# YulioTech/Yulio-Raytracer

Hardware: AMD Instinct MI355X
Metric: Mrays/s (Sponza stand-in 2048^2 64spp, closest+shadow queries) (higher is better)
Workload: dtype f32

## Files before the change

### yulio-raytracer_amd/csrc/device/bvh_build.cpp

```cpp
#include "bvh_build.h"

#include <float.h>
#include <math.h>
#include <stdlib.h>
#include <string.h>

#include <algorithm>
#include <stdexcept>

namespace yrt {

namespace {

struct Box {
  float lo[3], hi[3];
  void reset() {
    for (int k = 0; k < 3; ++k) { lo[k] = INFINITY; hi[k] = -INFINITY; }
  }
  void grow(const Box& b) {
    for (int k = 0; k < 3; ++k) { lo[k] = std::min(lo[k], b.lo[k]); hi[k] = std::max(hi[k], b.hi[k]); }
  }
  void growP(const float* p) {
    for (int k = 0; k < 3; ++k) { lo[k] = std::min(lo[k], p[k]); hi[k] = std::max(hi[k], p[k]); }
  }
  float area() const {
    const float dx = hi[0] - lo[0], dy = hi[1] - lo[1], dz = hi[2] - lo[2];
    if (!(dx >= 0 && dy >= 0 && dz >= 0)) return 0.f;
    return 2.f * (dx * dy + dy * dz + dz * dx);
  }
};

struct Prim {
  Box b;
  float c[3];
  int id;
};

struct Node2 {
  Box b[2];
  int idx[2], cnt[2];
};

struct Builder {
  std::vector<Prim> prims;
  std::vector<Node2> nodes;
#ifndef YRT_MAX_LEAF
#define YRT_MAX_LEAF 8
#endif
  int maxLeaf = YRT_MAX_LEAF;
#ifndef YRT_SAH_TRAV
#define YRT_SAH_TRAV 1.0f
#endif
  int medianDepth = 24;
  int maxDepthSeen = 0;

  Box bounds(int b, int e) const {
    Box bb;
    bb.reset();
    for (int i = b; i < e; ++i) bb.grow(prims[i].b);
    return bb;
  }

  int split(int b, int e, int depth, bool& makeLeaf) {
    const int n = e - b;
    makeLeaf = false;
    Box cb;
    cb.reset();
    for (int i = b; i < e; ++i) cb.growP(prims[i].c);
    int axis = 0;
    float ext = cb.hi[0] - cb.lo[0];
    for (int k = 1; k < 3; ++k)
      if (cb.hi[k] - cb.lo[k] > ext) { ext = cb.hi[k] - cb.lo[k]; axis = k; }
    if (!(ext > 0.f)) {
      if (n <= maxLeaf) { makeLeaf = true; return e; }
      return b + n / 2;
    }
    if (depth >= medianDepth) {
      const int m = b + n / 2;
      std::nth_element(prims.begin() + b, prims.begin() + m, prims.begin() + e,
                       [axis](const Prim& x, const Prim& y) { return x.c[axis] < y.c[axis]; });
      return m;
    }
    const int NB = 32;
    float bestCost = INFINITY;
    int bestAxis = -1, bestBin = -1;
    for (int ax = 0; ax < 3; ++ax) {
      const float lo = cb.lo[ax], hi = cb.hi[ax];
      if (!(hi > lo)) continue;
      const float scale = NB / (hi - lo);
      Box bb[NB];
      int cnt[NB] = {0};
      for (int k = 0; k < NB; ++k) bb[k].reset();
      for (int i = b; i < e; ++i) {
        int bin = std::min(NB - 1, (int)((prims[i].c[ax] - lo) * scale));
        cnt[bin]++;
        bb[bin].grow(prims[i].b);
      }
      float rightArea[NB];
      int rightCnt[NB];
      Box acc;
      acc.reset();
      int ac = 0;
      for (int k = NB - 1; k > 0; --k) {
        acc.grow(bb[k]);
        ac += cnt[k];
        rightArea[k] = acc.area();
        rightCnt[k] = ac;
      }
      acc.reset();
      ac = 0;
      for (int k = 0; k < NB - 1; ++k) {
        acc.grow(bb[k]);
        ac += cnt[k];
        if (ac == 0 || rightCnt[k + 1] == 0) continue;
        const float cost = acc.area() * ac + rightArea[k + 1] * rightCnt[k + 1];
        if (cost < bestCost) { bestCost = cost; bestAxis = ax; bestBin = k; }
      }
    }
    const float parentArea = bounds(b, e).area();
    const float leafCost = (float)n;
    const float splitCost = YRT_SAH_TRAV + (parentArea > 0.f ? bestCost / parentArea : (float)n);
    if (n <= maxLeaf && leafCost <= splitCost) { makeLeaf = true; return e; }
    if (bestAxis < 0) return b + n / 2;
    const float lo = cb.lo[bestAxis], hi = cb.hi[bestAxis];
    const float scale = NB / (hi - lo);
    auto mid = std::partition(prims.begin() + b, prims.begin() + e, [&](const Prim& p) {
      return std::min(NB - 1, (int)((p.c[bestAxis] - lo) * scale)) <= bestBin;
    });
    int m = (int)(mid - prims.begin());
    if (m <= b || m >= e) m = b + n / 2;
    return m;
  }

  void child(int b, int e, int depth, int& idx, int& cnt, Box& bb) {
    bb = bounds(b, e);
    const int n = e - b;
    if (n <= 2 && n < 32) { idx = b; cnt = n; return; }
    bool leaf = false;
    const int m = split(b, e, depth, leaf);
    if (leaf && n <= 31) { idx = b; cnt = n; return; }
    idx = inner(b, m, e, depth);
    cnt = 0;
  }

  int inner(int b, int m, int e, int depth) {
    if (depth > maxDepthSeen) maxDepthSeen = depth;
    const int ni = (int)nodes.size();
    nodes.emplace_back();
    int i0, c0, i1, c1;
    Box b0, b1;
    child(b, m, depth + 1, i0, c0, b0);
    child(m, e, depth + 1, i1, c1, b1);
    Node2& n = nodes[ni];
    n.b[0] = b0;
    n.b[1] = b1;
    n.idx[0] = i0; n.idx[1] = i1;
    n.cnt[0] = c0; n.cnt[1] = c1;
    return ni;
  }
};

#ifndef YRT_SBVH_ALPHA
#define YRT_SBVH_ALPHA 1e-5f
#endif
#ifndef YRT_SBVH_BUDGET
#define YRT_SBVH_BUDGET 0.5f
#endif
struct SRef {
  Box b;
  int id;
  float c(int k) const { return 0.5f * (b.lo[k] + b.hi[k]); }
};

Box clip_tri(const float* t, int axis, float lo, float hi) {
  Box r;
  r.reset();
  for (int e = 0; e < 3; ++e) {
    const float* p = t + 3 * e;
    const float* q = t + 3 * ((e + 1) % 3);
    const float pa = p[axis], qa = q[axis];
    if (pa >= lo && pa <= hi) r.growP(p);
    const float planes[2] = {lo, hi};
    for (float pl : planes) {
      if ((pa < pl && qa > pl) || (pa > pl && qa < pl)) {
        const double tt = ((double)pl - pa) / ((double)qa - pa);
        float x[3];
        for (int k = 0; k < 3; ++k) x[k] = (float)(p[k] + tt * ((double)q[k] - p[k]));
        x[axis] = pl;
        r.growP(x);
      }
    }
  }
  for (int k = 0; k < 3; ++k) {
    if (k == axis || !(r.hi[k] >= r.lo[k])) continue;
    const float pad = 4.0f * FLT_EPSILON * std::max(fabsf(r.lo[k]), fabsf(r.hi[k]));
    r.lo[k] -= pad;
    r.hi[k] += pad;
  }
  return r;
}

Box intersect(const Box& a, const Box& b) {
  Box r;
  for (int k = 0; k < 3; ++k) {
    r.lo[k] = std::max(a.lo[k], b.lo[k]);
    r.hi[k] = std::min(a.hi[k], b.hi[k]);
  }
  return r;
}

struct SplitBuilder {
  const std::vector<float>& v;
  std::vector<Node2> nodes;
  std::vector<int> leafIds;
  int maxLeaf = YRT_MAX_LEAF;
  int medianDepth = 24;
  float minOverlap = 0.f;
  size_t refBudget = 0, numRefs = 0;
  explicit SplitBuilder(const std::vector<float>& verts) : v(verts) {}

  static Box bounds(const std::vector<SRef>& r) {
    Box bb;
    bb.reset();
    for (const SRef& x : r) bb.grow(x.b);
    return bb;
  }

  void leaf(std::vector<SRef>& refs, int& idx, int& cnt) {
    idx = (int)leafIds.size();
    cnt = (int)refs.size();
    for (const SRef& x : refs) leafIds.push_back(x.id);
  }

  void child(std::vector<SRef>& refs, int depth, int& idx, int& cnt, Box& bb) {
    bb = bounds(refs);
    const int n = (int)refs.size();
    if (n <= 2) { leaf(refs, idx, cnt); return; }
    std::vector<SRef> L, R;
    const bool mkLeaf = split(refs, bb, depth, L, R);
    if (mkLeaf && n <= 31) { leaf(refs, idx, cnt); return; }
    if (mkLeaf) median(refs, bb, L, R);
    std::vector<SRef>().swap(refs);
    idx = inner(L, R, depth);
    cnt = 0;
  }

  int inner(std::vector<SRef>& L, std::vector<SRef>& R, int depth) {
    const int ni = (int)nodes.size();
    nodes.emplace_back();
    int i0, c0, i1, c1;
    Box b0, b1;
    child(L, depth + 1, i0, c0, b0);
    child(R, depth + 1, i1, c1, b1);
    Node2& nd = nodes[ni];
    nd.b[0] = b0;
    nd.b[1] = b1;
    nd.idx[0] = i0; nd.idx[1] = i1;
    nd.cnt[0] = c0; nd.cnt[1] = c1;
    return ni;
  }

  void median(std::vector<SRef>& refs, const Box& bb, std::vector<SRef>& L, std::vector<SRef>& R) {
    int axis = 0;
    for (int k = 1; k < 3; ++k)
      if (bb.hi[k] - bb.lo[k] > bb.hi[axis] - bb.lo[axis]) axis = k;
    const size_t m = refs.size() / 2;
    std::nth_element(refs.begin(), refs.begin() + m, refs.end(),
                     [axis](const SRef& x, const SRef& y) { return x.c(axis) < y.c(axis); });
    L.assign(refs.begin(), refs.begin() + m);
    R.assign(refs.begin() + m, refs.end());
  }

  bool split(std::vector<SRef>& refs, const Box& nodeBox, int depth, std::vector<SRef>& L, std::vector<SRef>& R) {
    const int n = (int)refs.size();
    Box cb;
    cb.reset();
    for (const SRef& x : refs) {
      const float c[3] = {x.c(0), x.c(1), x.c(2)};
      cb.growP(c);
    }
    if (depth >= medianDepth) {
      median(refs, cb, L, R);
      return false;
    }
    const int NB = 32;
    float objCost = INFINITY;
    int objAxis = -1, objBin = -1;
    Box objL, objR;
    for (int ax = 0; ax < 3; ++ax) {
      const float lo = cb.lo[ax], hi = cb.hi[ax];
      if (!(hi > lo)) continue;
      const float scale = NB / (hi - lo);
      Box bb[NB];
      int cnt[NB] = {0};
      for (int k = 0; k < NB; ++k) bb[k].reset();
      for (const SRef& x : refs) {
        const int bin = std::min(NB - 1, (int)((x.c(ax) - lo) * scale));
        cnt[bin]++;
        bb[bin].grow(x.b);
      }
      Box rightBox[NB];
      int rightCnt[NB];
      Box acc;
      acc.reset();
      int ac = 0;
      for (int k = NB - 1; k > 0; --k) {
        acc.grow(bb[k]);
        ac += cnt[k];
        rightBox[k] = acc;
        rightCnt[k] = ac;
      }
      acc.reset();
      ac = 0;
      for (int k = 0; k < NB - 1; ++k) {
        acc.grow(bb[k]);
        ac += cnt[k];
        if (ac == 0 || rightCnt[k + 1] == 0) continue;
        const float cost = acc.area() * ac + rightBox[k + 1].area() * rightCnt[k + 1];
        if (cost < objCost) {
          objCost = cost; objAxis = ax; objBin = k; objL = acc; objR = rightBox[k + 1];
        }
      }
    }
    float spCost = INFINITY;
    int spAxis = -1, spBin = -1;
    const float overlap = objAxis >= 0 ? intersect(objL, objR).area() : INFINITY;
    if (numRefs < refBudget && overlap > minOverlap) {
      for (int ax = 0; ax < 3; ++ax) {
        const float lo = nodeBox.lo[ax], hi = nodeBox.hi[ax];
        if (!(hi > lo)) continue;
        const float w = (hi - lo) / NB;
        Box bb[NB];
        int enter[NB] = {0}, exit[NB] = {0};
        for (int k = 0; k < NB; ++k) bb[k].reset();
        for (const SRef& x : refs) {
          const int b0 = std::max(0, std::min(NB - 1, (int)((x.b.lo[ax] - lo) / w)));
          const int b1 = std::max(b0, std::min(NB - 1, (int)((x.b.hi[ax] - lo) / w)));
          enter[b0]++;
          exit[b1]++;
          if (b0 == b1) {
            bb[b0].grow(x.b);
            continue;
          }
          const float* t = &v[(size_t)x.id * 9];
          for (int k = b0; k <= b1; ++k) {
            const float s0 = k == b0 ? x.b.lo[ax] : lo + k * w;
            const float s1 = k == b1 ? x.b.hi[ax] : lo + (k + 1) * w;
            const Box cbx = intersect(clip_tri(t, ax, s0, s1), x.b);
            if (cbx.hi[0] >= cbx.lo[0] && cbx.hi[1] >= cbx.lo[1] && cbx.hi[2] >= cbx.lo[2]) bb[k].grow(cbx);
          }
        }
        Box rightBox[NB];
        int rightCnt[NB];
        Box acc;
        acc.reset();
        int ac = 0;
        for (int k = NB - 1; k > 0; --k) {
          acc.grow(bb[k]);
          ac += exit[k];
          rightBox[k] = acc;
          rightCnt[k] = ac;
        }
        acc.reset();
        ac = 0;
        for (int k = 0; k < NB - 1; ++k) {
          acc.grow(bb[k]);
          ac += enter[k];
          if (ac == 0 || rightCnt[k + 1] == 0) continue;
          const float cost = acc.area() * ac + rightBox[k + 1].area() * rightCnt[k + 1];
          if (cost < spCost) { spCost = cost; spAxis = ax; spBin = k; }
        }
      }
    }
    const float parentArea = nodeBox.area();
    const float best = std::min(objCost, spCost);
    const float splitCost = YRT_SAH_TRAV + (parentArea > 0.f ? best / parentArea : (float)n);
    if (n <= maxLeaf && (float)n <= splitCost) return true;
    if (objAxis < 0 && spAxis < 0) return true;
    if (spAxis >= 0 && spCost < objCost) {
      const float lo = nodeBox.lo[spAxis], w = (nodeBox.hi[spAxis] - lo) / NB;
      const float plane = lo + (spBin + 1) * w;
      for (const SRef& x : refs) {
        if (x.b.hi[spAxis] <= plane) { L.push_back(x); continue; }
        if (x.b.lo[spAxis] >= plane) { R.push_back(x); continue; }
        const float* t = &v[(size_t)x.id * 9];
        const Box bl = intersect(clip_tri(t, spAxis, x.b.lo[spAxis], plane), x.b);
        const Box br = intersect(clip_tri(t, spAxis, plane, x.b.hi[spAxis]), x.b);
        const bool okL = bl.hi[0] >= bl.lo[0] && bl.hi[1] >= bl.lo[1] && bl.hi[2] >= bl.lo[2];
        const bool okR = br.hi[0] >= br.lo[0] && br.hi[1] >= br.lo[1] && br.hi[2] >= br.lo[2];
        if (okL) L.push_back(SRef{bl, x.id});
        if (okR) R.push_back(SRef{br, x.id});
        if (!okL && !okR) (x.c(spAxis) < plane ? L : R).push_back(x);
        if (okL && okR) numRefs++;
      }
      if (!L.empty() && !R.empty()) return false;
      refs.clear();
      for (auto* side : {&L, &R})
        for (const SRef& x : *side) refs.push_back(x);
      L.clear();
      R.clear();
      if (objAxis < 0) return true;
    }
    const float lo = cb.lo[objAxis], scale = NB / (cb.hi[objAxis] - lo);
    for (const SRef& x : refs)
      (std::min(NB - 1, (int)((x.c(objAxis) - lo) * scale)) <= objBin ? L : R).push_back(x);
    if (L.empty() || R.empty()) {
      L.clear();
      R.clear();
      return true;
    }
    return false;
  }
};

struct Ref {
  Box b;
  int idx, cnt;
};

struct Collapser {
  const std::vector<Node2>& in;
  std::vector<GpuNode> out;
  int maxStack = 0;
  explicit Collapser(const std::vector<Node2>& n) : in(n) {}

  int collapse(int n2, int stackAbove) {
    Ref ch[4];
    int k = 2;
    for (int j = 0; j < 2; ++j) ch[j] = Ref{in[n2].b[j], in[n2].idx[j], in[n2].cnt[j]};
    while (k < 4) {
      int best = -1;
      float bestArea = -1.f;
      for (int j = 0; j < k; ++j)
        if (ch[j].cnt == 0 && ch[j].b.area() > bestArea) { bestArea = ch[j].b.area(); best = j; }
      if (best < 0) break;
      const Node2& o = in[ch[best].idx];
      ch[best] = Ref{o.b[0], o.idx[0], o.cnt[0]};
      ch[k++] = Ref{o.b[1], o.idx[1], o.cnt[1]};
    }
    const int ni = (int)out.size();
    out.emplace_back();
    const int stackHere = stackAbove + (k - 1);
    if (stackHere > maxStack) maxStack = stackHere;
    int refs[4] = {-1, -1, -1, -1};
    for (int j = 0; j < k; ++j) {
      if (ch[j].cnt == 0) refs[j] = collapse(ch[j].idx, stackHere) << 5;
      else refs[j] = (ch[j].idx << 5) | ch[j].cnt;
    }
    GpuNode& g = out[ni];
    memset(&g, 0, sizeof(g));
    for (int j = 0; j < 4; ++j) {
      const bool v = j < k;
      const float L = INFINITY, H = -INFINITY;
      g.lox[j] = v ? ch[j].b.lo[0] : L; g.hix[j] = v ? ch[j].b.hi[0] : H;
      g.loy[j] = v ? ch[j].b.lo[1] : L; g.hiy[j] = v ? ch[j].b.hi[1] : H;
      g.loz[j] = v ? ch[j].b.lo[2] : L; g.hiz[j] = v ? ch[j].b.hi[2] : H;
      g.child[j] = refs[j];
    }
    return ni;
  }
};

}

void build_bvh(const std::vector<float>& v , const std::vector<uint32_t>& flags,
               int stackDepth, BvhResult& out, const std::vector<float>* v1) {
  const int N = (int)(v.size() / 9);
  out.nodes.clear();
  out.tris.clear();
  out.order.clear();
  if (N == 0) return;
  const int levels = (int)ceil(log2(std::max(1.0, N / 16.0)));
  const int medianDepth = std::max(0, std::min(28, (2 * stackDepth) / 3 - 2 - levels));
  std::vector<Node2> nodes2;
  std::vector<int> leafIds;
  const char* env = getenv("YRT_SBVH");
  const bool spatial = env && atoi(env) != 0 && !v1;
  if (N == 1) {
    Node2 n;
    n.b[0].reset();
    for (int k = 0; k < 3; ++k) n.b[0].growP(&v[3 * k]);
    if (v1)
      for (int k = 0; k < 3; ++k) n.b[0].growP(&(*v1)[3 * k]);
    n.b[1] = n.b[0];
    n.idx[0] = 0; n.cnt[0] = 1;
    n.idx[1] = 0; n.cnt[1] = 1;
    nodes2.push_back(n);
    leafIds.push_back(0);
  } else if (spatial) {
    SplitBuilder B(v);
    B.medianDepth = medianDepth;
    std::vector<SRef> refs(N);
    for (int i = 0; i < N; ++i) {
      refs[i].b.reset();
      for (int k = 0; k < 3; ++k) refs[i].b.growP(&v[(size_t)i * 9 + 3 * k]);
      refs[i].id = i;
    }
    const Box root = SplitBuilder::bounds(refs);
    B.minOverlap = YRT_SBVH_ALPHA * root.area();
    B.numRefs = (size_t)N;
    B.refBudget = (size_t)(N * (1.0 + YRT_SBVH_BUDGET));
    std::vector<SRef> L, R;
    bool leaf = B.split(refs, root, 0, L, R);
    if (leaf) B.median(refs, root, L, R);
    std::vector<SRef>().swap(refs);
    B.inner(L, R, 0);
    nodes2 = std::move(B.nodes);
    leafIds = std::move(B.leafIds);
  } else {
    Builder B;
    B.medianDepth = medianDepth;
    B.prims.resize(N);
    for (int i = 0; i < N; ++i) {
      Prim& p = B.prims[i];
      p.b.reset();
      for (int k = 0; k < 3; ++k) p.b.growP(&v[(size_t)i * 9 + 3 * k]);
      if (v1)
        for (int k = 0; k < 3; ++k) p.b.growP(&(*v1)[(size_t)i * 9 + 3 * k]);
      for (int k = 0; k < 3; ++k) p.c[k] = 0.5f * (p.b.lo[k] + p.b.hi[k]);
      p.id = i;
    }
    bool leaf = false;
    int m = B.split(0, N, 0, leaf);
    if (leaf || m <= 0 || m >= N) m = N / 2;
    B.inner(0, m, N, 0);
    nodes2 = std::move(B.nodes);
    leafIds.resize(N);
    for (int i = 0; i < N; ++i) leafIds[i] = B.prims[i].id;
  }
  Collapser C(nodes2);
  C.collapse(0, 0);
  out.maxDepth = C.maxStack;
  if (C.maxStack > stackDepth - 1)
    throw std::runtime_error("BVH traversal stack bound exceeds YRT_STACK_DEPTH");
  if (C.out.size() >= (size_t(1) << 25))
    throw std::runtime_error("BVH exceeds 2^25 nodes (32-bit node byte offsets)");
  if (leafIds.size() >= (size_t(1) << 26))
    throw std::runtime_error("BVH exceeds 2^26 leaf triangle references (child reference packing)");
  out.nodes = std::move(C.out);
  const size_t S = leafIds.size();
  out.order = leafIds;
  out.tris.resize(S);
  for (size_t i = 0; i < S; ++i) {
    const int id = leafIds[i];
    const float* t = &v[(size_t)id * 9];
    GpuTri& g = out.tris[i];
    g.v0[0] = t[0]; g.v0[1] = t[1]; g.v0[2] = t[2];
    g.e1[0] = t[0] - t[3]; g.e1[1] = t[1] - t[4]; g.e1[2] = t[2] - t[5];
    g.e2[0] = t[6] - t[0]; g.e2[1] = t[7] - t[1]; g.e2[2] = t[8] - t[2];
    int gid = id;
    uint32_t fl = flags[id];
    memcpy(&g.v0[3], &gid, 4);
    memcpy(&g.e1[3], &fl, 4);
    g.e2[3] = 0.f;
  }
}

}
```

### yulio-raytracer_amd/csrc/kernels/k_trace.h

```cpp
#pragma once

#include "yrt_camera.h"
#include "yrt_traverse.h"

namespace yrt {

#ifndef YRT_REFILL
#define YRT_REFILL 40
#endif
#ifndef YRT_REFILL_ANY
#define YRT_REFILL_ANY 32
#endif
#ifndef YRT_REFILL_PRIM
#define YRT_REFILL_PRIM YRT_REFILL
#endif
constexpr int kTriStep = 2;
#ifndef YRT_TRI_STEP_ANY
#define YRT_TRI_STEP_ANY kTriStep
#endif
#ifndef YRT_NODE_BIAS
#define YRT_NODE_BIAS 8
#endif
#ifndef YRT_NODE_BIAS_ANY
#define YRT_NODE_BIAS_ANY 20
#endif
#ifndef YRT_TRACE_WAVES
#define YRT_TRACE_WAVES 6
#endif
#ifndef YRT_TRACE_WAVES_PRIM
#define YRT_TRACE_WAVES_PRIM 5
#endif
#ifndef YRT_TRACE_WAVES_ANY
#define YRT_TRACE_WAVES_ANY 8
#endif
#ifdef YRT_PROFILE
#ifndef YRT_PROFILE_ANY
#define YRT_PROFILE_ANY 0
#endif
#define YRT_PROF(i, v) (ANY == (YRT_PROFILE_ANY != 0) ? (void)(prof[i] += (unsigned long long)(v)) : (void)0)
#else
#define YRT_PROF(i, v) ((void)0)
#endif

__device__ __forceinline__ void shadow_done(const ShadowFuse& sf, int* __restrict__ occOut, int q, bool occluded) {
  if (sf.contrib) {
    if (!occluded) {
      const float4 c = sf.contrib[q];
      const int tg = __float_as_int(c.w);
      float4* Lp = sf.pathL + tg;
      const float4 l = *Lp;
      *Lp = make_float4(l.x + c.x, l.y + c.y, l.z + c.z, l.w);
    }
  } else {
    occOut[q] = occluded ? 1 : 0;
  }
}

template <bool MOTION>
__device__ __forceinline__ GpuTri tri_at(const GpuTri* __restrict__ tris, const GpuTriMotion* __restrict__ tms,
                                         int slot, float time) {
  GpuTri t = tris[slot];
  if constexpr (MOTION) {
    const GpuTriMotion m = tms[slot];
    const float p0x = t.v0[0] + time * m.m0[0], p0y = t.v0[1] + time * m.m0[1], p0z = t.v0[2] + time * m.m0[2];
    const float p1x = m.p1[0] + time * m.m1[0], p1y = m.p1[1] + time * m.m1[1], p1z = m.p1[2] + time * m.m1[2];
    const float p2x = m.p2[0] + time * m.m2[0], p2y = m.p2[1] + time * m.m2[1], p2z = m.p2[2] + time * m.m2[2];
    t.v0[0] = p0x; t.v0[1] = p0y; t.v0[2] = p0z;
    t.e1[0] = p0x - p1x; t.e1[1] = p0y - p1y; t.e1[2] = p0z - p1z;
    t.e2[0] = p2x - p0x; t.e2[1] = p2y - p0y; t.e2[2] = p2z - p0z;
  }
  return t;
}

template <bool ANY, bool MOTION, int PRIM = 0>
__global__ __launch_bounds__(YRT_TRACE_BLOCK) __attribute__((amdgpu_waves_per_eu(
    ANY ? YRT_TRACE_WAVES_ANY : PRIM ? YRT_TRACE_WAVES_PRIM : YRT_TRACE_WAVES))) void k_trace(
    SceneView sv, const float4* __restrict__ org,
                                                         const float4* __restrict__ dir,
                                                         const unsigned* __restrict__ counts, int numSegs,
                                                         int segCap, float4* __restrict__ hitOut,
                                                         int* __restrict__ occOut, int* __restrict__ spillBuf,
                                                         ShadowFuse sf, const float* __restrict__ rayTime,
                                                         PrimaryRays pr) {
  static_assert(!PRIM || (!ANY && !MOTION), "camera rays: closest hit, static scenes");
  constexpr int kLds = ANY ? YRT_LDS_STACK_ANY : PRIM ? YRT_LDS_STACK_PRIM : YRT_LDS_STACK;
  __shared__ int lstack[kLds * YRT_TRACE_BLOCK];
  __shared__ QMap qm;
  unsigned n;
  if constexpr (PRIM) {
    n = (unsigned)pr.bi.numPixels * (unsigned)const_ref(pr.fv.rp).spp;
  } else {
    qmap_load(qm, counts, numSegs);
    n = qm.pre[YRT_QSEGS];
  }
  const int lane = lane_id();
  const unsigned wavesPerBlock = YRT_TRACE_BLOCK / 64;
  const unsigned gw = blockIdx.x * wavesPerBlock + (threadIdx.x >> 6);
  const unsigned numWaves = gridDim.x * wavesPerBlock;
  unsigned chunk = (n + numWaves - 1) / numWaves;
  chunk = chunk < 64u ? 64u : chunk;
  unsigned next = gw * chunk;
  const unsigned end = min(n, next + chunk);
  if (next >= end) return;

  const GpuQNode* __restrict__ qnodes = sv.qnodes;
  const GpuTri* __restrict__ tris = sv.tris;
  int* stack = lstack + threadIdx.x;
  const size_t spillStride = (size_t)gridDim.x * YRT_TRACE_BLOCK;
  int* __restrict__ spill = spillBuf + blockIdx.x * YRT_TRACE_BLOCK + threadIdx.x;

  bool has = false;
  int q = 0, sp = 0, curIdx = 0, curCnt = 0, pendIdx = 0, pendCnt = 0;
#define YRT_SLOT(i) ((((i) & (kLds - 1))) * YRT_TRACE_BLOCK)
#define YRT_POP_READ(e_)                                                          \
  do {                                                                            \
    e_ = (unsigned)stack[YRT_SLOT(sp)];                                           \
    if (sp >= kLds) stack[YRT_SLOT(sp)] = spill[(size_t)(sp - kLds) * spillStride]; \
  } while (0)
#define YRT_PUSH(e)                                                               \
  do {                                                                            \
    if (sp >= kLds) spill[(size_t)(sp - kLds) * spillStride] = stack[YRT_SLOT(sp)]; \
    stack[YRT_SLOT(sp)] = (e);                                                    \
    sp += 1;                                                                      \
  } while (0)
#define YRT_POP()                                                                 \
  do {                                                                            \
    if (sp == 0) {                                                                \
      curCnt = -1;                                                                \
    } else {                                                                      \
      sp -= 1;                                                                    \
      unsigned e_;                                                                \
      YRT_POP_READ(e_);                                                           \
      curIdx = (int)(e_ >> 5);                                                    \
      curCnt = (int)(e_ & 31u);                                                   \
    }                                                                             \
  } while (0)
  float4 ro = make_float4(0.f, 0.f, 0.f, 0.f), rd = ro, ri = ro, rc = ro;
  float rtime = 0.f;
  Hit best;
  best.t = best.u = best.v = 0.f;
  best.tri = -1;
  float bestDen = 1.f;
  q = -1;
  auto prim_store = [&]() {
    const bool hitp = best.tri >= 0;
    if (!hitp) {
      const float* mL = pr.fv.rp->missL;
      pr.pathL[q] = make_float4(mL[0], mL[1], mL[2], mL[3]);
    }
    const int seg = qseg_of((unsigned)q);
    unsigned long long m = ballot(hitp);
    while (m) {
      const int l0 = __ffsll((long long)m) - 1;
      const int seg0 = __builtin_amdgcn_readlane(seg, l0);
      const unsigned long long sub = ballot(hitp && seg == seg0);
      unsigned base = 0;
      if (lane == l0) base = atomicAdd(pr.counts + (size_t)seg0 * YRT_QCSTRIDE, (unsigned)__popcll(sub));
      base = (unsigned)__builtin_amdgcn_readlane((int)base, l0);
      if (hitp && seg == seg0) {
        const unsigned slot = (unsigned)seg0 * (unsigned)pr.segCap + base + lanes_below(sub);
        pr.qPath[slot] = q;
        pr.qOrg[slot] = ro;
        pr.qDir[slot] = rd;
        hitOut[slot] = make_float4(best.t, best.u / bestDen, best.v / bestDen, __int_as_float(best.tri));
      }
      m &= ~sub;
    }
  };
#define YRT_STORE_HIT()                                                                              \
  do {                                                                                               \
    if constexpr (PRIM)                                                                              \
      prim_store();                                                                                  \
    else                                                                                             \
      hitOut[q] = make_float4(best.t, best.u / bestDen, best.v / bestDen, __int_as_float(best.tri)); \
    q = -1;                                                                                          \
  } while (0)

#ifdef YRT_PROFILE
  unsigned long long prof[8] = {0, 0, 0, 0, 0, 0, 0, 0};
#endif
  while (true) {
    if (has && curCnt < 0 && pendCnt == 0) {
      if (ANY) shadow_done(sf, occOut, q, false);
      has = false;
    }
    const unsigned long long idle = ballot(!has);
    const int nIdle = __popcll(idle);
    YRT_PROF(0, 1);
    YRT_PROF(1, 64 - nIdle);
    if (nIdle >= (ANY ? YRT_REFILL_ANY : PRIM ? YRT_REFILL_PRIM : YRT_REFILL)) {
      if (next < end) {
        const unsigned li = next + lanes_below(idle);
        if (!has) {
          if (!ANY && q >= 0) YRT_STORE_HIT();
          if (li < end) {
            if constexpr (PRIM) {
              const YRT_CONST GpuRenderParams& rp = const_ref(pr.fv.rp);
              const int p = (int)li;
              const int smp = fastdiv(p, pr.bi.divPixels);
              int x = 0, y = 0, f = 0;
              const bool valid = batch_pixel(rp, pr.bi, p - smp * pr.bi.numPixels, x, y, f) && rp.maxDepth > 0 &&
                                 !(1.0f < rp.minContribution);
              if (valid) {
                const int rec = pr.fv.pixelSets[(size_t)y * rp.width + x] * rp.spp + smp;
                const float fx = (float(x) + samp(pr.fv, 0, rec)) * rp.rcpWidth;
                const float fy = (float(y) + samp(pr.fv, 1, rec)) * rp.rcpHeight;
                const float lx = samp(pr.fv, 2, rec), ly = samp(pr.fv, 3, rec);
                V3 o3 = v3s(0.f), d3 = v3s(0.f);
                for (bool todo = true; todo;) {
                  const int f0 = __builtin_amdgcn_readfirstlane(f);
                  if (f == f0) {
                    const YRT_CONST GpuCamera& cam = const_ref(pr.fv.cam + f0);
                    camera_ray<false>(cam, fx, fy, o3, d3, lx, ly);
                    todo = false;
                  }
                }
                ro = make_float4(o3.x, o3.y, o3.z, 0.f);
                rd = make_float4(d3.x, d3.y, d3.z, __int_as_float(0x7f800000));
                q = p;
              } else {
                const float z = opaque_zero();
                pr.pathL[p] = make_float4(z, z, z, z);
                q = -1;
                ro = make_float4(0.f, 0.f, 0.f, 1.f);
                rd = make_float4(0.f, 0.f, 1.f, 0.f);
              }
            } else {
            q = qmap_phys(qm, segCap, li);
            ro = org[q];
            rd = dir[q];
            if (MOTION) rtime = rayTime[q];
            }
            ri = make_float4(safe_inv(rd.x), safe_inv(rd.y), safe_inv(rd.z), 0.f);
            ri.w = __int_as_float(plane_offsets(ri.x, ri.y, ri.z));
            {
              V3 oi;
              float mg;
              ray_slab_consts(v3(ro.x, ro.y, ro.z), v3(ri.x, ri.y, ri.z), oi, mg);
              rc = make_float4(oi.x, oi.y, oi.z, mg);
            }
            best.t = rd.w;
            best.u = best.v = 0.f;
            best.tri = -1;
            bestDen = 1.f;
            sp = 0;
            curIdx = 0;
            curCnt = 0;
            pendCnt = 0;
            has = rd.w >= ro.w;
            if (!has) {
              if (ANY) shadow_done(sf, occOut, q, false);
            }
          }
        }
        next += (unsigned)nIdle;
      } else if (nIdle == 64) {
        if (!ANY && q >= 0) YRT_STORE_HIT();
        if constexpr (PRIM) {
          const YRT_CONST GpuRenderParams& rp = const_ref(pr.fv.rp);
          unsigned t = 0;
          if (rp.maxDepth > 0 && !(1.0f < rp.minContribution)) {
            for (unsigned b = gw * chunk; b < end; b += 64) {
              const unsigned p = b + (unsigned)lane;
              bool v = false;
              if (p < end) {
                const int smp = fastdiv((int)p, pr.bi.divPixels);
                int x, y, f;
                v = batch_pixel(rp, pr.bi, (int)p - smp * pr.bi.numPixels, x, y, f);
              }
              t += (unsigned)__popcll(ballot(v));
            }
          }
          if (lane == 0 && t) atomicAdd(pr.traced, t);
        }
#ifdef YRT_PROFILE
        if (lane == 0)
          for (int k = 0; k < 8; ++k) atomicAdd(&g_traceProfile[k], prof[k]);
#endif
        break;
      }
    }
    RayPre r;
    r.org = v3(ro.x, ro.y, ro.z);
    r.dir = v3(rd.x, rd.y, rd.z);
    r.inv = v3(ri.x, ri.y, ri.z);
    r.tnear = ro.w;
    r.tfar = rd.w;
    r.oi = v3(rc.x, rc.y, rc.z);
    r.margin = rc.w;

    const unsigned long long hasB = ballot(has);
#define YRT_NNODE() __popcll(ballot(curCnt == 0) & hasB)
#define YRT_NBLOCKED() __popcll(ballot(max(pendCnt, curCnt) > 0) & ~ballot(curCnt == 0) & hasB)
    const int nNode = YRT_NNODE();
    const int nBlocked = YRT_NBLOCKED();
    if (nNode * 4 > nBlocked * (ANY ? YRT_NODE_BIAS_ANY : YRT_NODE_BIAS)) {
     while (true) {
      YRT_PROF(2, 1);
      YRT_PROF(3, __popcll(ballot(has && curCnt == 0)));
      if (has && curCnt == 0) {
        float t[4];
        int c[4];
        box4_quant<ANY>(r, __float_as_int(ri.w), best.t, t, c, qnodes, curIdx);
        if (!ANY) sort4(t, c);
        else sort3_far(t, c);
        const float MISS = __int_as_float(ANY ? 0xff800000 : 0x7f800000);
#define YRT_HIT(x) (ANY ? (x) > MISS : (x) < MISS)
        if (sp + 3 <= kLds) {
          const int h3 = YRT_HIT(t[3]), h2 = YRT_HIT(t[2]), h1 = YRT_HIT(t[1]);
          stack[YRT_SLOT(sp)] = c[3];
          stack[YRT_SLOT(sp + h3)] = c[2];
          stack[YRT_SLOT(sp + h3 + h2)] = c[1];
          sp += h3 + h2 + h1;
        } else {
          if (YRT_HIT(t[3])) YRT_PUSH(c[3]);
          if (YRT_HIT(t[2])) YRT_PUSH(c[2]);
          if (YRT_HIT(t[1])) YRT_PUSH(c[1]);
        }
        if (YRT_HIT(t[0])) {
          curIdx = c[0] >> 5;
          curCnt = c[0] & 31;
        } else {
          YRT_POP();
        }
#undef YRT_HIT
        if (curCnt > 0 && pendCnt == 0) {
          pendIdx = curIdx;
          pendCnt = curCnt;
          YRT_POP();
        }
      }
      const int nNode2 = YRT_NNODE();
      const int nBlocked2 = YRT_NBLOCKED();
      if (!(nNode2 * 4 > nBlocked2 * (ANY ? YRT_NODE_BIAS_ANY : YRT_NODE_BIAS))) break;
     }
    } else {
      const bool usePend = pendCnt > 0;
      const int lIdx = usePend ? pendIdx : curIdx;
      const int lCnt = !has ? 0 : usePend ? pendCnt : (curCnt > 0 ? curCnt : 0);
#ifdef YRT_PROFILE
      {
        const int lc_ = min(lCnt, ANY ? YRT_TRI_STEP_ANY : kTriStep);
        int mx = lc_;
        for (int o = 32; o > 0; o >>= 1) mx = max(mx, __shfl_xor(mx, o, 64));
        int sm = lc_;
        for (int o = 32; o > 0; o >>= 1) sm += __shfl_xor(sm, o, 64);
        YRT_PROF(4, mx > 0 ? 1 : 0);
        YRT_PROF(5, mx);
        YRT_PROF(6, sm);
      }
#endif
      bool found = false;
      const int lTake = min(lCnt, ANY ? YRT_TRI_STEP_ANY : kTriStep);
      if (!ANY) {
        if (lTake > 0) {
          GpuTri tt[kTriStep];
#pragma unroll
          for (int k = 0; k < kTriStep; ++k) tt[k] = tri_at<MOTION>(tris, sv.triMotion, lIdx + min(k, lTake - 1), rtime);
#pragma unroll
          for (int k = 0; k < kTriStep; ++k) {
            float t, U, V, absDen;
            const bool g = tri_test_g(tt[k], r, t, U, V, absDen);
            const int gid = __float_as_int(tt[k].v0[3]);
            const bool tie = (t == best.t) & (best.tri >= 0) & (gid < best.tri);
            const bool ok = g & (t > r.tnear) & ((t < best.t + 0.0f) | tie);
            if (ok & (k < lTake)) {
              best.t = t; best.u = U; best.v = V; bestDen = absDen; best.tri = gid;
            }
          }
        }
      } else {
        for (int i = 0; i < lTake && !found; ++i) {
          const GpuTri tr = tri_at<MOTION>(tris, sv.triMotion, lIdx + i, rtime);
          float t, U, V, absDen;
          found = tri_test_t(tr, r, r.tfar, t, U, V, absDen);
        }
      }
      if (lCnt > 0) {
        if (usePend) {
          pendIdx += lTake;
          pendCnt -= lTake;
        } else if (curCnt > lTake) {
          curIdx += lTake;
          curCnt -= lTake;
        } else {
          YRT_POP();
        }
      }
      if (ANY && found) {
        shadow_done(sf, occOut, q, true);
        has = false;
      }
    }
  }
}

#undef YRT_SLOT
#undef YRT_POP_READ
#undef YRT_PUSH
#undef YRT_POP
#undef YRT_STORE_HIT
#undef YRT_NNODE
#undef YRT_NBLOCKED
#undef YRT_PROF

}
```

### yulio-raytracer_amd/csrc/kernels/yrt_traverse.h

```cpp
#pragma once

#include "../common/yrt_gpu_types.h"
#include "../common/yrt_math.h"
#include "../common/yrt_qnode.h"

#ifndef YRT_STACK_DEPTH
#define YRT_STACK_DEPTH 64
#endif
#ifndef YRT_LDS_STACK
#define YRT_LDS_STACK 16
#endif
static_assert((YRT_LDS_STACK & (YRT_LDS_STACK - 1)) == 0, "YRT_LDS_STACK must be a power of two");
#ifndef YRT_LDS_STACK_ANY
#define YRT_LDS_STACK_ANY 16
#endif
static_assert((YRT_LDS_STACK_ANY & (YRT_LDS_STACK_ANY - 1)) == 0, "YRT_LDS_STACK_ANY must be a power of two");
#ifndef YRT_LDS_STACK_PRIM
#define YRT_LDS_STACK_PRIM 16
#endif
static_assert((YRT_LDS_STACK_PRIM & (YRT_LDS_STACK_PRIM - 1)) == 0, "YRT_LDS_STACK_PRIM must be a power of two");
#define YRT_LDS_STACK_MIN2 (YRT_LDS_STACK < YRT_LDS_STACK_ANY ? YRT_LDS_STACK : YRT_LDS_STACK_ANY)
#define YRT_LDS_STACK_MIN (YRT_LDS_STACK_MIN2 < YRT_LDS_STACK_PRIM ? YRT_LDS_STACK_MIN2 : YRT_LDS_STACK_PRIM)
#ifndef YRT_TRACE_BLOCK
#define YRT_TRACE_BLOCK 64
#endif

namespace yrt {

struct Hit {
  float t, u, v;
  int tri;
};

#ifndef YRT_BOX_ROBUST
#define YRT_BOX_ROBUST 1.0000152587890625f
#endif

__device__ __forceinline__ float safe_inv(float d) {
  return rcp_rn(fabsf(d) > 1e-20f ? d : copysignf(1e-20f, d));
}

struct RayPre {
  V3 org, dir, inv;
  float tnear, tfar;
  V3 oi;
  float margin;
};

__device__ __forceinline__ void ray_slab_consts(const V3& org, const V3& inv, V3& oi, float& margin) {
  oi = v3(org.x * inv.x, org.y * inv.y, org.z * inv.z);
  margin = fmaxf(fmaxf(fabsf(oi.x), fabsf(oi.y)), fabsf(oi.z)) * 2.384185791015625e-07f;
}

__device__ __forceinline__ void box4(const GpuNode* __restrict__ np, const RayPre& r, float tmax, float t[4],
                                     int c[4]) {
  typedef float f2 __attribute__((ext_vector_type(2)));
  const float4* q = (const float4*)np;
  const float4 lx = q[0], hx = q[1], ly = q[2], hy = q[3], lz = q[4], hz = q[5];
  const int4 ch = *(const int4*)(q + 6);
  const f2 ox = {r.org.x, r.org.x}, oy = {r.org.y, r.org.y}, oz = {r.org.z, r.org.z};
  const f2 ix = {r.inv.x, r.inv.x}, iy = {r.inv.y, r.inv.y}, iz = {r.inv.z, r.inv.z};
  f2 lx01 = (f2{lx.x, lx.y} - ox) * ix, lx23 = (f2{lx.z, lx.w} - ox) * ix;
  f2 hx01 = (f2{hx.x, hx.y} - ox) * ix, hx23 = (f2{hx.z, hx.w} - ox) * ix;
  f2 ly01 = (f2{ly.x, ly.y} - oy) * iy, ly23 = (f2{ly.z, ly.w} - oy) * iy;
  f2 hy01 = (f2{hy.x, hy.y} - oy) * iy, hy23 = (f2{hy.z, hy.w} - oy) * iy;
  f2 lz01 = (f2{lz.x, lz.y} - oz) * iz, lz23 = (f2{lz.z, lz.w} - oz) * iz;
  f2 hz01 = (f2{hz.x, hz.y} - oz) * iz, hz23 = (f2{hz.z, hz.w} - oz) * iz;
  const float INF = __int_as_float(0x7f800000);
#define YRT_FLAT_IN(LO_, O, HI_) (((LO_) <= (O) && (O) <= (HI_)) ? -INF : INF)
#define YRT_FLAT_AXIS(D, O, LO, HI, L01, L23, H01, H23)               \
  if (!(fabsf(D) > 1e-20f)) {                                         \
    L01 = f2{YRT_FLAT_IN(LO.x, O, HI.x), YRT_FLAT_IN(LO.y, O, HI.y)}; \
    L23 = f2{YRT_FLAT_IN(LO.z, O, HI.z), YRT_FLAT_IN(LO.w, O, HI.w)}; \
    H01 = H23 = f2{INF, INF};                                         \
  }
  YRT_FLAT_AXIS(r.dir.x, r.org.x, lx, hx, lx01, lx23, hx01, hx23)
  YRT_FLAT_AXIS(r.dir.y, r.org.y, ly, hy, ly01, ly23, hy01, hy23)
  YRT_FLAT_AXIS(r.dir.z, r.org.z, lz, hz, lz01, lz23, hz01, hz23)
#undef YRT_FLAT_AXIS
#undef YRT_FLAT_IN
#define YRT_CHILD(k, LX, HX, LY, HY, LZ, HZ, CH)                                                          \
  do {                                                                                                    \
    const float nn = fmaxf(fmaxf(fminf(LX, HX), fminf(LY, HY)), fmaxf(fminf(LZ, HZ), r.tnear));          \
    const float ff = fminf(fminf(fmaxf(LX, HX), fmaxf(LY, HY)), fminf(fmaxf(LZ, HZ), tmax));             \
    t[k] = ((nn <= ff * YRT_BOX_ROBUST) && (CH) != -1) ? nn : INF;                                        \
    c[k] = (CH);                                                                                          \
  } while (0)
  YRT_CHILD(0, lx01.x, hx01.x, ly01.x, hy01.x, lz01.x, hz01.x, ch.x);
  YRT_CHILD(1, lx01.y, hx01.y, ly01.y, hy01.y, lz01.y, hz01.y, ch.y);
  YRT_CHILD(2, lx23.x, hx23.x, ly23.x, hy23.x, lz23.x, hz23.x, ch.z);
  YRT_CHILD(3, lx23.y, hx23.y, ly23.y, hy23.y, lz23.y, hz23.y, ch.w);
#undef YRT_CHILD
}

__device__ __forceinline__ int plane_offsets(float ix, float iy, float iz) {
  return ((__float_as_uint(ix) >> 27) & 16) | ((__float_as_uint(iy) >> 19) & (16 << 8)) |
         ((__float_as_uint(iz) >> 11) & (16 << 16));
}

struct QNodeData {
  float4 h;
  int4 ch;
  uint4 pa;
  uint2 pb;
};
__device__ __forceinline__ QNodeData qnode_load(const GpuQNode* __restrict__ base, int nodeIdx) {
  const char* b0 = (const char*)base + ((unsigned)nodeIdx << 6);
  QNodeData d;
  d.h = *(const float4*)b0;
  d.ch = *(const int4*)(b0 + 16);
  d.pa = *(const uint4*)(b0 + 32);
  d.pb = *(const uint2*)(b0 + 48);
  return d;
}
template <bool ANY>
__device__ __forceinline__ void box4_qdata(const QNodeData& d, const RayPre& r, int planeOff, float tmax, float t[4],
                                           int c[4]) {
  typedef float f2 __attribute__((ext_vector_type(2)));
  const float4 h = d.h;
  const int4 ch = d.ch;
  const uint4 pa = d.pa;
  const uint2 pb = d.pb;
  const uint32_t ex = __float_as_uint(h.w);
  const float sx = __uint_as_float((ex & 0xffu) << 23) * r.inv.x;
  const float sy = __uint_as_float(((ex >> 8) & 0xffu) << 23) * r.inv.y;
  const float sz = __uint_as_float(((ex >> 16) & 0xffu) << 23) * r.inv.z;
  const float ax = __builtin_fmaf(h.x, r.inv.x, -r.oi.x);
  const float ay = __builtin_fmaf(h.y, r.inv.y, -r.oi.y);
  const float az = __builtin_fmaf(h.z, r.inv.z, -r.oi.z);
  const bool hx = (planeOff & 16) != 0, hy = (planeOff & (16 << 8)) != 0, hz = (planeOff & (16 << 16)) != 0;
  const uint32_t nwx = hx ? pa.y : pa.x, fwx = hx ? pa.x : pa.y;
  const uint32_t nwy = hy ? pa.w : pa.z, fwy = hy ? pa.z : pa.w;
  const uint32_t nwz = hz ? pb.y : pb.x, fwz = hz ? pb.x : pb.y;
#define YRT_QB(w, k) ((float)(((w) >> (8 * (k))) & 0xffu))
#define YRT_QSLAB(W, S, A, k0, k1) __builtin_elementwise_fma((f2{YRT_QB(W, k0), YRT_QB(W, k1)}), (f2{S, S}), (f2{A, A}))
  const f2 nx01 = YRT_QSLAB(nwx, sx, ax, 0, 1), nx23 = YRT_QSLAB(nwx, sx, ax, 2, 3);
  const f2 fx01 = YRT_QSLAB(fwx, sx, ax, 0, 1), fx23 = YRT_QSLAB(fwx, sx, ax, 2, 3);
  const f2 ny01 = YRT_QSLAB(nwy, sy, ay, 0, 1), ny23 = YRT_QSLAB(nwy, sy, ay, 2, 3);
  const f2 fy01 = YRT_QSLAB(fwy, sy, ay, 0, 1), fy23 = YRT_QSLAB(fwy, sy, ay, 2, 3);
  const f2 nz01 = YRT_QSLAB(nwz, sz, az, 0, 1), nz23 = YRT_QSLAB(nwz, sz, az, 2, 3);
  const f2 fz01 = YRT_QSLAB(fwz, sz, az, 0, 1), fz23 = YRT_QSLAB(fwz, sz, az, 2, 3);
#undef YRT_QSLAB
#undef YRT_QB
  const float MISS = __int_as_float(ANY ? 0xff800000 : 0x7f800000);
#define YRT_CHILD(k, NX, FX, NY, FY, NZ, FZ, CH)                                            \
  do {                                                                                      \
    float nn, ff, a_, b_;                                                                   \
    asm("v_max_f32 %0, %1, %2" : "=v"(a_) : "v"(NZ), "v"(r.tnear));                         \
    asm("v_max3_f32 %0, %1, %2, %3" : "=v"(nn) : "v"(NX), "v"(NY), "v"(a_));                \
    asm("v_min_f32 %0, %1, %2" : "=v"(b_) : "v"(FZ), "v"(tmax));                            \
    asm("v_min3_f32 %0, %1, %2, %3" : "=v"(ff) : "v"(FX), "v"(FY), "v"(b_));                \
    t[k] = ((int)(nn <= __builtin_fmaf(ff, YRT_BOX_ROBUST, r.margin)) & (int)((CH) != -1)) ? nn : MISS; \
    c[k] = (CH);                                                                            \
  } while (0)
  YRT_CHILD(0, nx01.x, fx01.x, ny01.x, fy01.x, nz01.x, fz01.x, ch.x);
  YRT_CHILD(1, nx01.y, fx01.y, ny01.y, fy01.y, nz01.y, fz01.y, ch.y);
  YRT_CHILD(2, nx23.x, fx23.x, ny23.x, fy23.x, nz23.x, fz23.x, ch.z);
  YRT_CHILD(3, nx23.y, fx23.y, ny23.y, fy23.y, nz23.y, fz23.y, ch.w);
#undef YRT_CHILD
}
template <bool ANY>
__device__ __forceinline__ void box4_quant(const RayPre& r, int planeOff, float tmax, float t[4], int c[4],
                                           const GpuQNode* __restrict__ base, int nodeIdx) {
  box4_qdata<ANY>(qnode_load(base, nodeIdx), r, planeOff, tmax, t, c);
}

__device__ __forceinline__ void sort4(float t[4], int c[4]) {
#define YRT_CSWAP(a, b)                          \
  do {                                           \
    const bool sw = t[b] < t[a];                 \
    const float ta = sw ? t[b] : t[a];           \
    const float tb = sw ? t[a] : t[b];           \
    const int ca = sw ? c[b] : c[a];             \
    const int cb = sw ? c[a] : c[b];             \
    t[a] = ta; t[b] = tb; c[a] = ca; c[b] = cb;  \
  } while (0)
  YRT_CSWAP(0, 1);
  YRT_CSWAP(2, 3);
  YRT_CSWAP(0, 2);
  YRT_CSWAP(1, 3);
  YRT_CSWAP(1, 2);
#undef YRT_CSWAP
}

__device__ __forceinline__ void sort3_far(float t[4], int c[4]) {
#define YRT_CSWAP_D(a, b)                        \
  do {                                           \
    const bool sw = t[b] > t[a];                 \
    const float ta = sw ? t[b] : t[a];           \
    const float tb = sw ? t[a] : t[b];           \
    const int ca = sw ? c[b] : c[a];             \
    const int cb = sw ? c[a] : c[b];             \
    t[a] = ta; t[b] = tb; c[a] = ca; c[b] = cb;  \
  } while (0)
  YRT_CSWAP_D(0, 1);
  YRT_CSWAP_D(2, 3);
  YRT_CSWAP_D(0, 2);
#undef YRT_CSWAP_D
}

__device__ __forceinline__ V3 tri_cross(const V3& a, const V3& b) {
  return v3(a.y * b.z - a.z * b.y, a.z * b.x - a.x * b.z, a.x * b.y - a.y * b.x);
}
__device__ __forceinline__ float tri_dot(const V3& a, const V3& b) { return a.x * b.x + a.y * b.y + a.z * b.z; }

__device__ __forceinline__ bool tri_test_g(const GpuTri& tr, const RayPre& r, float& t, float& U_, float& V_,
                                           float& absDen_) {
  V3 v0 = v3(tr.v0[0], tr.v0[1], tr.v0[2]);
  V3 e1 = v3(tr.e1[0], tr.e1[1], tr.e1[2]);
  V3 e2 = v3(tr.e2[0], tr.e2[1], tr.e2[2]);
  V3 Ng = tri_cross(e1, e2);
  V3 C = v0 - r.org;
  V3 R = tri_cross(r.dir, C);
  float den = tri_dot(Ng, r.dir);
  float absDen = fabsf(den);
  float sgn = den < 0.0f ? -1.0f : 1.0f;
  float U = tri_dot(R, e2) * sgn;
  float V = tri_dot(R, e1) * sgn;
  bool ok = (den != 0.0f) & (U >= 0.0f) & (V >= 0.0f) & (U + V <= absDen);
  int flags = __float_as_int(tr.e1[3]);
  ok &= !((flags & 1) && !(den > 0.0f));
  float T = tri_dot(Ng, C) * sgn;
  t = T / absDen;
  U_ = U;
  V_ = V;
  absDen_ = absDen;
  return ok;
}

__device__ __forceinline__ bool tri_test_t(const GpuTri& tr, const RayPre& r, float tfar, float& t, float& U_,
                                           float& V_, float& absDen_) {
  V3 v0 = v3(tr.v0[0], tr.v0[1], tr.v0[2]);
  V3 e1 = v3(tr.e1[0], tr.e1[1], tr.e1[2]);
  V3 e2 = v3(tr.e2[0], tr.e2[1], tr.e2[2]);
  V3 Ng = tri_cross(e1, e2);
  V3 C = v0 - r.org;
  V3 R = tri_cross(r.dir, C);
  float den = tri_dot(Ng, r.dir);
  float absDen = fabsf(den);
  float sgn = den < 0.0f ? -1.0f : 1.0f;
  float U = tri_dot(R, e2) * sgn;
  float V = tri_dot(R, e1) * sgn;
  bool ok = (den != 0.0f) & (U >= 0.0f) & (V >= 0.0f) & (U + V <= absDen);
  int flags = __float_as_int(tr.e1[3]);
  ok &= !((flags & 1) && !(den > 0.0f));
  float T = tri_dot(Ng, C) * sgn;
  t = T / absDen;
  ok &= (t > r.tnear) & (t < tfar);
  U_ = U;
  V_ = V;
  absDen_ = absDen;
  return ok;
}

template <bool ANY>
__device__ __forceinline__ Hit traverse(const GpuNode* __restrict__ nodes, const GpuTri* __restrict__ tris,
                                        const RayPre& r, int* __restrict__ stack ) {
  (void)stack;
  Hit best;
  best.t = r.tfar;
  best.u = best.v = 0.0f;
  best.tri = -1;
  if (!(r.tfar >= r.tnear)) return best;
  int pst[YRT_STACK_DEPTH];
  int sp = 0;
  int cur = 0;
  while (true) {
    if ((cur & 31) == 0) {
      float t[4];
      int c[4];
      box4(nodes + (cur >> 5), r, best.t, t, c);
      sort4(t, c);
      const float INF = __int_as_float(0x7f800000);
      if (t[3] < INF) pst[sp++] = c[3];
      if (t[2] < INF) pst[sp++] = c[2];
      if (t[1] < INF) pst[sp++] = c[1];
      if (t[0] < INF) {
        cur = c[0];
        continue;
      }
    } else {
      const int idx = cur >> 5, cnt = cur & 31;
      for (int i = 0; i < cnt; ++i) {
        const GpuTri tr = tris[idx + i];
        float t, U, V, absDen;
        bool ok = tri_test_t(tr, r, ANY ? r.tfar : best.t + 0.0f, t, U, V, absDen);
        int gid = __float_as_int(tr.v0[3]);
        if (ANY) {
          if (ok) {
            best.t = t; best.u = U / absDen; best.v = V / absDen; best.tri = gid;
            return best;
          }
        } else {
          if (!ok && best.tri >= 0 && t == best.t && gid < best.tri) {
            float t2, U2, V2, a2;
            ok = tri_test_t(tr, r, r.tfar, t2, U2, V2, a2);
          }
          if (ok) {
            best.t = t; best.u = U / absDen; best.v = V / absDen; best.tri = gid;
          }
        }
      }
    }
    if (sp == 0) break;
    cur = pst[--sp];
  }
  return best;
}

}
```

Before: 7402.

## Add optional LDS cache of top BVH nodes with breadth-first node reordering

Reorders the collapsed BVH so the first N nodes form a breadth-first top tree, and optionally copies those top quantized nodes into shared memory at kernel start, reading them from LDS instead of global memory during traversal. When enabled, the per-thread LDS stack ring shrinks to make room. The top-node cache defaults to 0 for all kernel variants, so only the host-side node reorder (default top of 85 nodes) is active by default. Also adds spill-count profiling hooks. The reorder changes memory locality of upper nodes, and the LDS path trades stack depth for node-fetch latency.

```diff
diff --git a/yulio-raytracer_amd/csrc/device/bvh_build.cpp b/yulio-raytracer_amd/csrc/device/bvh_build.cpp
--- a/yulio-raytracer_amd/csrc/device/bvh_build.cpp
+++ b/yulio-raytracer_amd/csrc/device/bvh_build.cpp
@@ -461,6 +461,36 @@
   }
 };
 
+#ifndef YRT_TOP_NODES_MAX
+#define YRT_TOP_NODES_MAX 85
+#endif
+void top_breadth_first(std::vector<GpuNode>& nodes, int topMax) {
+  const int n = (int)nodes.size();
+  const int T = std::min(n, topMax);
+  if (T <= 1) return;
+  auto inner = [](int c) { return c != -1 && (c & 31) == 0; };
+  std::vector<int> top = {0};
+  top.reserve(T);
+  for (size_t w = 0; w < top.size() && (int)top.size() < T; ++w)
+    for (int k = 0; k < 4 && (int)top.size() < T; ++k) {
+      const int c = nodes[top[w]].child[k];
+      if (inner(c)) top.push_back(c >> 5);
+    }
+  std::vector<int> newIdx(n, -1);
+  for (size_t i = 0; i < top.size(); ++i) newIdx[top[i]] = (int)i;
+  int next = (int)top.size();
+  for (int i = 0; i < n; ++i)
+    if (newIdx[i] < 0) newIdx[i] = next++;
+  std::vector<GpuNode> out(n);
+  for (int i = 0; i < n; ++i) {
+    GpuNode g = nodes[i];
+    for (int k = 0; k < 4; ++k)
+      if (inner(g.child[k])) g.child[k] = newIdx[g.child[k] >> 5] << 5;
+    out[newIdx[i]] = g;
+  }
+  nodes.swap(out);
+}
+
 }
 
 void build_bvh(const std::vector<float>& v , const std::vector<uint32_t>& flags,
@@ -538,6 +568,8 @@
   if (leafIds.size() >= (size_t(1) << 26))
     throw std::runtime_error("BVH exceeds 2^26 leaf triangle references (child reference packing)");
   out.nodes = std::move(C.out);
+  const char* topEnv = getenv("YRT_TOP_NODES_MAX");
+  top_breadth_first(out.nodes, topEnv ? atoi(topEnv) : YRT_TOP_NODES_MAX);
   const size_t S = leafIds.size();
   out.order = leafIds;
   out.tris.resize(S);
diff --git a/yulio-raytracer_amd/csrc/kernels/k_trace.h b/yulio-raytracer_amd/csrc/kernels/k_trace.h
--- a/yulio-raytracer_amd/csrc/kernels/k_trace.h
+++ b/yulio-raytracer_amd/csrc/kernels/k_trace.h
@@ -40,6 +40,11 @@
 #define YRT_PROF(i, v) (ANY == (YRT_PROFILE_ANY != 0) ? (void)(prof[i] += (unsigned long long)(v)) : (void)0)
 #else
 #define YRT_PROF(i, v) ((void)0)
+#endif
+#if defined(YRT_PROFILE) && defined(YRT_PROFILE_SPILL)
+#define YRT_SPILL_COUNT() ((void)(profSpill += 1))
+#else
+#define YRT_SPILL_COUNT() ((void)0)
 #endif
 
 __device__ __forceinline__ void shadow_done(const ShadowFuse& sf, int* __restrict__ occOut, int q, bool occluded) {
@@ -83,8 +88,12 @@
                                                          ShadowFuse sf, const float* __restrict__ rayTime,
                                                          PrimaryRays pr) {
   static_assert(!PRIM || (!ANY && !MOTION), "camera rays: closest hit, static scenes");
-  constexpr int kLds = ANY ? YRT_LDS_STACK_ANY : PRIM ? YRT_LDS_STACK_PRIM : YRT_LDS_STACK;
+  constexpr int kTop = ANY ? YRT_TOP_LDS_ANY : PRIM ? YRT_TOP_LDS_PRIM : YRT_TOP_LDS;
+  constexpr int kLds = ANY ? YRT_RING_ANY : PRIM ? YRT_RING_PRIM : YRT_RING_CLOSEST;
+  static_assert(kTop == 0 || kLds * YRT_TRACE_BLOCK * 4 + kTop * YRT_TOP_STRIDE <= 16 * 64 * 4,
+                "stack ring + top nodes exceed the 16-entry ring's LDS");
   __shared__ int lstack[kLds * YRT_TRACE_BLOCK];
+  __shared__ uint4 topNodes[kTop > 0 ? kTop * (YRT_TOP_STRIDE / 16) : 1];
   __shared__ QMap qm;
   unsigned n;
   if constexpr (PRIM) {
@@ -101,9 +110,16 @@
   chunk = chunk < 64u ? 64u : chunk;
   unsigned next = gw * chunk;
   const unsigned end = min(n, next + chunk);
+  if (YRT_TRACE_BLOCK == 64 && next >= end) return;
+  const GpuQNode* __restrict__ qnodes = sv.qnodes;
+  if constexpr (kTop > 0) {
+    const int pieces = 4 * min(kTop, sv.numNodes);
+    for (int i = (int)threadIdx.x; i < pieces; i += YRT_TRACE_BLOCK)
+      topNodes[(i >> 2) * (YRT_TOP_STRIDE / 16) + (i & 3)] = ((const uint4*)qnodes)[i];
+    __syncthreads();
+  }
   if (next >= end) return;
 
-  const GpuQNode* __restrict__ qnodes = sv.qnodes;
   const GpuTri* __restrict__ tris = sv.tris;
   int* stack = lstack + threadIdx.x;
   const size_t spillStride = (size_t)gridDim.x * YRT_TRACE_BLOCK;
@@ -119,7 +135,10 @@
   } while (0)
 #define YRT_PUSH(e)                                                               \
   do {                                                                            \
-    if (sp >= kLds) spill[(size_t)(sp - kLds) * spillStride] = stack[YRT_SLOT(sp)]; \
+    if (sp >= kLds) {                                                             \
+      spill[(size_t)(sp - kLds) * spillStride] = stack[YRT_SLOT(sp)];             \
+      YRT_SPILL_COUNT();                                                          \
+    }                                                                             \
     stack[YRT_SLOT(sp)] = (e);                                                    \
     sp += 1;                                                                      \
   } while (0)
@@ -178,6 +197,7 @@
 
 #ifdef YRT_PROFILE
   unsigned long long prof[8] = {0, 0, 0, 0, 0, 0, 0, 0};
+  int profSpill = 0;
 #endif
   while (true) {
     if (has && curCnt < 0 && pendCnt == 0) {
@@ -274,6 +294,10 @@
           if (lane == 0 && t) atomicAdd(pr.traced, t);
         }
 #ifdef YRT_PROFILE
+#ifdef YRT_PROFILE_SPILL
+        for (int o = 32; o > 0; o >>= 1) profSpill += __shfl_xor(profSpill, o, 64);
+        YRT_PROF(7, profSpill);
+#endif
         if (lane == 0)
           for (int k = 0; k < 8; ++k) atomicAdd(&g_traceProfile[k], prof[k]);
 #endif
@@ -298,10 +322,20 @@
      while (true) {
       YRT_PROF(2, 1);
       YRT_PROF(3, __popcll(ballot(has && curCnt == 0)));
+#ifndef YRT_PROFILE_SPILL
+      YRT_PROF(7, __popcll(ballot(has && curCnt == 0 && curIdx < kTop)));
+#endif
       if (has && curCnt == 0) {
         float t[4];
         int c[4];
-        box4_quant<ANY>(r, __float_as_int(ri.w), best.t, t, c, qnodes, curIdx);
+        QNodeData nd;
+        if constexpr (kTop > 0) {
+          if (curIdx >= kTop) nd = qnode_load(qnodes, curIdx);
+          else nd = qnode_load_lds(topNodes, curIdx);
+        } else {
+          nd = qnode_load(qnodes, curIdx);
+        }
+        box4_qdata<ANY>(nd, r, __float_as_int(ri.w), best.t, t, c);
         if (!ANY) sort4(t, c);
         else sort3_far(t, c);
         const float MISS = __int_as_float(ANY ? 0xff800000 : 0x7f800000);
@@ -403,5 +437,6 @@
 #undef YRT_NNODE
 #undef YRT_NBLOCKED
 #undef YRT_PROF
+#undef YRT_SPILL_COUNT
 
 }
diff --git a/yulio-raytracer_amd/csrc/kernels/yrt_traverse.h b/yulio-raytracer_amd/csrc/kernels/yrt_traverse.h
--- a/yulio-raytracer_amd/csrc/kernels/yrt_traverse.h
+++ b/yulio-raytracer_amd/csrc/kernels/yrt_traverse.h
@@ -19,8 +19,29 @@
 #define YRT_LDS_STACK_PRIM 16
 #endif
 static_assert((YRT_LDS_STACK_PRIM & (YRT_LDS_STACK_PRIM - 1)) == 0, "YRT_LDS_STACK_PRIM must be a power of two");
-#define YRT_LDS_STACK_MIN2 (YRT_LDS_STACK < YRT_LDS_STACK_ANY ? YRT_LDS_STACK : YRT_LDS_STACK_ANY)
-#define YRT_LDS_STACK_MIN (YRT_LDS_STACK_MIN2 < YRT_LDS_STACK_PRIM ? YRT_LDS_STACK_MIN2 : YRT_LDS_STACK_PRIM)
+#ifndef YRT_TOP_LDS
+#define YRT_TOP_LDS 0
+#endif
+#ifndef YRT_TOP_LDS_ANY
+#define YRT_TOP_LDS_ANY 0
+#endif
+#ifndef YRT_TOP_LDS_PRIM
+#define YRT_TOP_LDS_PRIM 0
+#endif
+#ifndef YRT_LDS_STACK_TOP
+#define YRT_LDS_STACK_TOP 8
+#endif
+static_assert((YRT_LDS_STACK_TOP & (YRT_LDS_STACK_TOP - 1)) == 0, "YRT_LDS_STACK_TOP must be a power of two");
+#ifndef YRT_TOP_STRIDE
+#define YRT_TOP_STRIDE 80
+#endif
+static_assert(YRT_TOP_STRIDE >= 64 && YRT_TOP_STRIDE % 16 == 0, "LDS node stride: 16-B pieces of a 64-B node");
+#define YRT_RING_OF(K_, RING_) ((K_) > 0 ? YRT_LDS_STACK_TOP : (RING_))
+#define YRT_RING_CLOSEST YRT_RING_OF(YRT_TOP_LDS, YRT_LDS_STACK)
+#define YRT_RING_ANY YRT_RING_OF(YRT_TOP_LDS_ANY, YRT_LDS_STACK_ANY)
+#define YRT_RING_PRIM YRT_RING_OF(YRT_TOP_LDS_PRIM, YRT_LDS_STACK_PRIM)
+#define YRT_LDS_STACK_MIN2 (YRT_RING_CLOSEST < YRT_RING_ANY ? YRT_RING_CLOSEST : YRT_RING_ANY)
+#define YRT_LDS_STACK_MIN (YRT_LDS_STACK_MIN2 < YRT_RING_PRIM ? YRT_LDS_STACK_MIN2 : YRT_RING_PRIM)
 #ifndef YRT_TRACE_BLOCK
 #define YRT_TRACE_BLOCK 64
 #endif
@@ -111,6 +132,23 @@
   d.ch = *(const int4*)(b0 + 16);
   d.pa = *(const uint4*)(b0 + 32);
   d.pb = *(const uint2*)(b0 + 48);
+  return d;
+}
+__device__ __forceinline__ QNodeData qnode_load_lds(const uint4* top, int nodeIdx) {
+  unsigned i = (unsigned)nodeIdx;
+#if YRT_TOP_STRIDE == 80
+  asm("v_lshl_add_u32 %0, %1, 2, %1" : "=v"(i) : "v"(nodeIdx));
+#else
+  i *= YRT_TOP_STRIDE / 16;
+#endif
+  const uint4* p = top + i;
+  const uint4 a = p[0];
+  QNodeData d;
+  d.h = make_float4(__uint_as_float(a.x), __uint_as_float(a.y), __uint_as_float(a.z), __uint_as_float(a.w));
+  const uint4 b = p[1];
+  d.ch = make_int4((int)b.x, (int)b.y, (int)b.z, (int)b.w);
+  d.pa = p[2];
+  d.pb = *(const uint2*)(p + 3);
   return d;
 }
 template <bool ANY>
```

Result: no change. 7436 (median of 6 runs) (+0.5%).
